# wgurecky/CORRLA_RS

Measured on AMD Instinct MI355X. Metric: RSVD GFLOP/s on 16k x 16k f32 rank-128, higher is better.
Workload: dtype f32

## Files before the change

### corrla_rs_amd/csrc/core_svd_plan.hpp

```cpp
#pragma once
#include <algorithm>
#include <cmath>
#include <cstddef>
#include <cstdint>
#include <cstring>
#include <limits>

#if defined(__HIPCC__)
#include <hip/hip_runtime.h>
#define CORRLA_HD __host__ __device__
#else
#define CORRLA_HD
#endif

namespace corrla {
namespace k {

constexpr size_t kLdsMaxBytes = (size_t)160 * 1024;

constexpr int kJmcMaxSweeps = 40;
constexpr int kJmcLanes = 16;
CORRLA_HD constexpr int jmc_rows(int nc, int lanes) { return nc * 2 * lanes; }
CORRLA_HD constexpr int jmc_pitch(int nc, int esz, int lanes) {
  return lanes == 8 ? (jmc_rows(nc, 8) + ((nc % 2 == 0) ? 16 : 0))
                    : (esz == 4 ? (jmc_rows(nc, 16) + ((nc % 2 == 0) ? 32 : 0)) : jmc_rows(nc, 16));
}
CORRLA_HD constexpr size_t jmc_lds_bytes(int nc, int b, int esz, int lanes) {
  return (size_t)2 * (2 * b) * jmc_pitch(nc, esz, lanes) * esz + (size_t)2 * b * esz + 64;
}

constexpr int kRingProcPad = 72;
constexpr int kReplayLanes = 16;
CORRLA_HD inline size_t jacobi_ring_w_lds_bytes(int l, int rs, size_t esz) {
  const int n2 = (l + 1) & ~1;
  const int nproc = n2 / 2;
  return (size_t)2 * nproc * rs * esz + (size_t)n2 * (esz + sizeof(int)) + (size_t)2 * nproc * esz + 64;
}
inline int jacobi_ring_e(int64_t l, int esz) { return l <= 64 ? 8 : (l <= 96 ? 12 : (l <= 128 ? 16 : (esz == 4 ? 20 : 18))); }

inline size_t jacobi_block_round_lds_bytes(int rows_pad, size_t esz) {
  return (size_t)(2 * 16 * (rows_pad + 1) + 7 * 16 * 17 + 32) * esz + 16 * sizeof(int) + 64;
}
inline size_t jacobi_finish_lds_bytes(int l, size_t esz) { return (size_t)(l + 2) * esz + (size_t)(l + 2) * sizeof(int) + 64; }

}

inline bool jmc_geometry(int64_t l, int esz, int jmc_max_b, int local, int np_force, int* nc_out, int* np_out, int* b_out) {
  if (l < 2 || l > 288) return false;
  const int nc = (int)((l + 2 * k::kJmcLanes - 1) / (2 * k::kJmcLanes));
  auto width = [&](int np_) {
    int bb = (int)((l + 2 * np_ - 1) / (2 * np_));
    return local ? (bb + 3) / 4 * 4 : bb + (bb & 1);
  };
  int np = np_force;
  if (np <= 0) {
    np = 2;
    while (np < 128 && (width(np) > jmc_max_b || k::jmc_lds_bytes(nc, width(np), esz, k::kJmcLanes) > k::kLdsMaxBytes)) ++np;
  }
  const int b = width(np);
  if (np < 1 || b < 2 || b > 32 || k::jmc_lds_bytes(nc, b, esz, k::kJmcLanes) > k::kLdsMaxBytes) return false;
  *nc_out = nc;
  *np_out = np;
  *b_out = b;
  return true;
}

enum class CoreSvd {
  kRing,
  kMultiWg,
  kBlock,
  kHost,
};
struct CoreSvdKnobs {
  const char* mode = nullptr;
  bool host_svd = false;
  int jmc_min_l = 96;
  int jmc_max_b = 24;
  int jmc_local = 1;
  int jmc_np = 0;
  int jmc_sweeps_f32 = 10, jmc_sweeps_f64 = 13;
  bool jmc_force_v = false;
  bool strict = false;
  int block_sweeps = 12, ring_sweeps = 40;
  int block_inner = 1;
};
struct CoreSvdState {
  int sweeps_hint = 0;
  int extra_sweeps = 0;
  bool force_v = false;
};

struct CoreSvdPlan {
  CoreSvd family = CoreSvd::kHost;
  int ring_e = 0;
  double tol = 0;
  double tol_early = 0;
  double floor2 = 0;
  struct MultiWg {
    int nc, np, b;
    int local;
    int rp;
    int nblocks, ncols_pad;
    unsigned step_threads;
    size_t step_lds;
    size_t ws_bytes;
    size_t fin_lds;
    unsigned other_grid;
    int force_v;
    int nsw;
    int group, max_sweeps;
  } mc = {};
  struct Block {
    int nb;
    int cols_pad, rows_pad;
    size_t ws_bytes;
    size_t round_lds;
    int max_sweeps, inner;
    size_t fin_lds;
  } blk = {};
  struct Ring {
    unsigned block;
    size_t lds;
    int max_sw;
    size_t rot_bytes, rank_bytes;
    unsigned replay_grid;
  } ring = {};
};

inline CoreSvdPlan core_svd_plan(int esz, int64_t l, int64_t k, const CoreSvdKnobs& kn, const CoreSvdState& st, bool optimistic) {
  auto is = [&](const char* m) { return kn.mode && std::strcmp(kn.mode, m) == 0; };
  CoreSvdPlan p;
  CoreSvdPlan::MultiWg& g = p.mc;
  const int e = k::jacobi_ring_e(l, esz);
  if ((!kn.mode || is("mc")) && !kn.host_svd && (is("mc") || l >= kn.jmc_min_l) &&
      jmc_geometry(l, esz, kn.jmc_max_b, kn.jmc_local, kn.jmc_np, &g.nc, &g.np, &g.b))
    p.family = CoreSvd::kMultiWg;
  else if (kn.host_svd || is("host") || l > 1024)
    return p;
  else if (!is("block") && l >= 2 && l <= 144 && k::jacobi_ring_w_lds_bytes((int)l, 8 * e, (size_t)esz) <= k::kLdsMaxBytes)
    p.family = CoreSvd::kRing;
  else
    p.family = CoreSvd::kBlock;

  const double eps = esz == 4 ? (double)std::numeric_limits<float>::epsilon() : std::numeric_limits<double>::epsilon();
  p.tol = std::sqrt((double)l) * eps;
  p.tol_early = kn.strict && p.family != CoreSvd::kBlock ? p.tol : std::sqrt(eps);
  p.floor2 = (double)l * eps * eps;
  switch (p.family) {
    case CoreSvd::kMultiWg: {
      g.local = kn.jmc_local;
      g.rp = k::jmc_pitch(g.nc, esz, k::kJmcLanes);
      g.nblocks = 2 * g.np;
      g.ncols_pad = g.nblocks * g.b;
      g.step_threads = (unsigned)((g.b * k::kJmcLanes + 63) / 64 * 64);
      g.step_lds = k::jmc_lds_bytes(g.nc, g.b, esz, k::kJmcLanes);
      g.ws_bytes = (size_t)g.rp * g.ncols_pad * esz;
      g.fin_lds = k::jacobi_finish_lds_bytes((int)l, (size_t)esz);
      g.other_grid = ((unsigned)(l * k) * 16 + 255) / 256;
      g.force_v = (!optimistic || st.force_v || kn.jmc_force_v) ? 1 : 0;
      const int nsw_default = std::max(1, esz == 4 ? kn.jmc_sweeps_f32 : kn.jmc_sweeps_f64);
      g.nsw = std::min(k::kJmcMaxSweeps, (st.sweeps_hint > 0 ? std::min(nsw_default, st.sweeps_hint + 2) : nsw_default) + st.extra_sweeps);
      g.group = 8;
      g.max_sweeps = k::kJmcMaxSweeps;
      break;
    }
    case CoreSvd::kBlock: {
      CoreSvdPlan::Block& b = p.blk;
      b.nb = (int)(2 * ((l + 15) / 16));
      b.cols_pad = b.nb * 8;
      b.rows_pad = (int)((l + 15) / 16 * 16);
      b.ws_bytes = (size_t)b.rows_pad * b.cols_pad * esz;
      b.round_lds = k::jacobi_block_round_lds_bytes(b.rows_pad, (size_t)esz);
      b.max_sweeps = kn.block_sweeps;
      b.inner = kn.block_inner;
      b.fin_lds = k::jacobi_finish_lds_bytes((int)l, (size_t)esz);
      break;
    }
    case CoreSvd::kRing: {
      CoreSvdPlan::Ring& r = p.ring;
      const int np = (int)((l + 1) / 2), n2 = 2 * np;
      p.ring_e = e;
      r.block = (unsigned)(np * 8);
      r.lds = k::jacobi_ring_w_lds_bytes((int)l, 8 * e, (size_t)esz);
      r.max_sw = kn.ring_sweeps;
      r.rot_bytes = (size_t)r.max_sw * n2 * k::kRingProcPad * (2 * (size_t)esz);
      r.rank_bytes = sizeof(int) * (size_t)n2;
      r.replay_grid = (unsigned)((l + 256 / k::kReplayLanes - 1) / (256 / k::kReplayLanes));
      break;
    }
    case CoreSvd::kHost: break;
  }
  return p;
}
inline CoreSvdPlan core_svd_plan(int esz, int64_t l, const CoreSvdKnobs& kn) { return core_svd_plan(esz, l, l, kn, CoreSvdState{}, true); }

}
```

### corrla_rs_amd/csrc/core_svd_stage.hpp

```cpp
#pragma once
#include "core_svd_plan.hpp"
#include "hip_backend.hpp"

namespace corrla {

template <class T>
struct CoreSvdCall {
  const Skinny<T>& c;
  int64_t l, k;
  Skinny<T>&m1, &m2;
  T* s_dev;
  void* conv_status;
};

namespace core_svd_stage {

template <class T>
using RingEs = std::integer_sequence<int, 8, 12, 16, sizeof(T) == 4 ? 20 : 18>;
constexpr int kMaxNc = 9;

template <class T>
inline void set_lds_limits() {
  for_each_of(RingEs<T>{}, [](auto e) { lds_limit((const void*)k::jacobi_ring_w_kernel<T, decltype(e)::value, 8>, k::kLdsMaxBytes); });
  lds_limit((const void*)k::jacobi_block_round_kernel<T>, k::kLdsMaxBytes);
  for_each_nt<kMaxNc>([](auto nc) { lds_limit((const void*)k::jmc_step_kernel<T, decltype(nc)::value, k::kJmcLanes>, k::kLdsMaxBytes); });
}

template <class T>
inline void multi_wg(HipDev& dev, const CoreSvdCall<T>& a, const CoreSvdPlan& plan) {
  const CoreSvdPlan::MultiWg& p = plan.mc;
  const int l = (int)a.l;
  T* wj = (T*)dev.alloc_bytes(p.ws_bytes);
  T* vj = (T*)dev.alloc_bytes(p.ws_bytes);
  k::JmcCtl* ctl = (k::JmcCtl*)dev.alloc_bytes(sizeof(k::JmcCtl));
  k::CholStatus* st = a.conv_status ? (k::CholStatus*)a.conv_status : (k::CholStatus*)dev.alloc_bytes(sizeof(k::CholStatus));
  hipLaunchKernelGGL((k::jmc_init_kernel<T>), dim3(1), dim3(1024), 0, dev.stream, (const T*)a.c.p, a.c.ld, l, wj, vj, p.rp,
                     p.ncols_pad, p.force_v, ctl);
  const T tol = (T)plan.tol, tol_early = (T)plan.tol_early, floor2 = (T)plan.floor2;
  auto enqueue_sweeps = [&](int s0, int s1) {
    for (int sw = s0; sw < s1; ++sw)
      for (int step = 0; step < p.nblocks - 1; ++step)
        with_nt<kMaxNc>(p.nc, [&](auto nc) {
          hipLaunchKernelGGL((k::jmc_step_kernel<T, decltype(nc)::value, k::kJmcLanes>), dim3((unsigned)p.np), dim3(p.step_threads),
                             p.step_lds, dev.stream, wj, vj, p.b, p.nblocks, step, sw, step == 0 ? 1 : 0, tol, tol_early, floor2,
                             ctl, p.local);
        });
    CORRLA_HIP(hipGetLastError());
  };
  auto finish = [&](int nsw) {
    hipLaunchKernelGGL((k::jmc_finish_kernel<T>), dim3(1), dim3(1024), p.fin_lds, dev.stream, (const T*)wj, (const T*)vj, p.rp, l,
                       nsw, (const k::JmcCtl*)ctl, a.m1.p, a.m1.ld, a.m2.p, a.m2.ld, a.s_dev, (int)a.k, st);
    hipLaunchKernelGGL((k::jmc_other_factor_kernel<T>), dim3(p.other_grid), dim3(256), 0, dev.stream, (const T*)a.c.p, a.c.ld, l,
                       (int)a.k, (const T*)a.m2.p, a.m2.ld, (const T*)a.s_dev, (const k::JmcCtl*)ctl, a.m1.p, a.m1.ld);
    CORRLA_HIP(hipGetLastError());
  };
  if (a.conv_status) {
    const int nsw = p.nsw;
    enqueue_sweeps(0, nsw);
    finish(nsw);
    if (env_int("CORRLA_DEBUG", 0)) {
      k::JmcCtl hd;
      CORRLA_HIP(hipMemcpyAsync(&hd, ctl, sizeof(hd), hipMemcpyDeviceToHost, dev.stream));
      dev.sync();
      int used = 0;
      while (used < nsw && hd.rot[used] && hd.big[used]) ++used;
      std::fprintf(stderr, "[corrla] jacobi_svd (multi-workgroup, %d sweeps enqueued, %s) l=%d np=%d b=%d nc=%d sweeps run=%d rounds(wg0)=%llu "
                           "cycles/round=%.0f ns/round=%.0f (%.0f MHz)\n", nsw, hd.with_v ? "V accumulated" : "W only", l, p.np, p.b, p.nc, std::min(used + 1, nsw),
                   hd.rounds, hd.rounds ? (double)hd.clk / hd.rounds : 0.0, hd.rounds ? 10.0 * hd.wall / hd.rounds : 0.0,
                   hd.wall ? 100.0 * hd.clk / hd.wall : 0.0);
      if (hd.steps)
        std::fprintf(stderr, "[corrla]   per step (wg0, us): load %.2f norms %.2f rounds %.2f store %.2f total %.2f over %llu steps\n",
                     0.01 * hd.t_load / hd.steps, 0.01 * hd.t_norm / hd.steps, 0.01 * hd.wall / hd.steps,
                     0.01 * hd.t_store / hd.steps, 0.01 * hd.t_total / hd.steps, hd.steps);
      if (hd.steps > 1)
        std::fprintf(stderr, "[corrla]   span first-start..last-end over all workgroups: %.2f us per step\n",
                     0.01 * hd.t_span / (hd.steps - 1));
    }
    return;
  }
  int done = 0;
  k::JmcCtl h;
  while (done < p.max_sweeps) {
    const int s1 = std::min(p.max_sweeps, done + p.group);
    enqueue_sweeps(done, s1);
    CORRLA_HIP(hipMemcpyAsync(&h, ctl, sizeof(h), hipMemcpyDeviceToHost, dev.stream));
    dev.sync();
    bool conv = false;
    for (int s_ = 0; s_ < s1; ++s_) conv = conv || !(h.rot[s_] && h.big[s_]);
    done = s1;
    if (conv || h.bad) break;
  }
  if (h.bad) throw Error(ST_ENUMERIC, "non-finite core matrix in small SVD");
  finish(done);
  if (env_int("CORRLA_DEBUG", 0)) {
    int used = 0;
    while (used < done && h.rot[used] && h.big[used]) ++used;
    std::fprintf(stderr, "[corrla] jacobi_svd (multi-workgroup) l=%d np=%d b=%d sweeps=%d\n", l, p.np, p.b, used + 1);
  }
}

template <class T>
inline void finite_check(HipDev& dev, const CoreSvdCall<T>& a) {
  int* bad = a.conv_status ? nullptr : dev.alloc_flags(1);
  hipLaunchKernelGGL((k::core_finite_check_kernel<T>), dim3(1), dim3(1024), 0, dev.stream, (const T*)a.c.p, a.c.ld, (int)a.l,
                     (k::CholStatus*)a.conv_status, bad);
  CORRLA_HIP(hipGetLastError());
  if (bad) {
    int h = 0;
    dev.read_flags(bad, 1, &h);
    if (h) throw Error(ST_ENUMERIC, "non-finite core matrix in small SVD");
  }
}

template <class T>
inline void block(HipDev& dev, const CoreSvdCall<T>& a, const CoreSvdPlan& plan) {
  const CoreSvdPlan::Block& p = plan.blk;
  const int64_t ld = p.rows_pad;
  T* wj = (T*)dev.alloc_bytes(p.ws_bytes);
  T* vj = (T*)dev.alloc_bytes(p.ws_bytes);
  k::JacobiCtl* ctl = (k::JacobiCtl*)dev.alloc_bytes(sizeof(k::JacobiCtl));
  hipLaunchKernelGGL((k::jacobi_init_kernel<T>), dim3(64), dim3(256), 0, dev.stream, (const T*)a.c.p, a.c.ld, (int)a.l, wj, ld, vj,
                     ld, p.cols_pad, p.rows_pad, ctl);
  for (int sw = 0; sw < p.max_sweeps; ++sw) {
    for (int round = 0; round < p.nb - 1; ++round)
      hipLaunchKernelGGL((k::jacobi_block_round_kernel<T>), dim3(p.nb / 2), dim3(256), p.round_lds, dev.stream, wj, ld, vj, ld,
                         p.rows_pad, p.nb, round, p.inner, ctl);
    hipLaunchKernelGGL(k::jacobi_sweep_end_kernel, dim3(1), dim3(1), 0, dev.stream, ctl, (float)plan.tol_early);
  }
  hipLaunchKernelGGL((k::jacobi_finish_kernel<T>), dim3(1), dim3(1024), p.fin_lds, dev.stream, (const T*)wj, ld, (const T*)vj,
                     ld, (int)a.l, a.m1.p, a.m1.ld, a.m2.p, a.m2.ld, a.s_dev, (int)a.k);
  CORRLA_HIP(hipGetLastError());
  if (env_int("CORRLA_DEBUG", 0)) {
    k::JacobiCtl h;
    CORRLA_HIP(hipMemcpyAsync(&h, ctl, sizeof(h), hipMemcpyDeviceToHost, dev.stream));
    dev.sync();
    std::fprintf(stderr, "[corrla] block jacobi l=%d nb=%d sweeps=%u done=%u\n", (int)a.l, p.nb, h.sweeps, h.done);
  }
}

template <class T>
inline void ring(HipDev& dev, const CoreSvdCall<T>& a, const CoreSvdPlan& plan) {
  static_assert(sizeof(k::RotEntry<T>) == 2 * sizeof(T), "CoreSvdPlan::Ring::rot_bytes");
  const CoreSvdPlan::Ring& p = plan.ring;
  int* info = (int*)dev.alloc_bytes(sizeof(int) * 4);
  k::RotEntry<T>* rot = (k::RotEntry<T>*)dev.alloc_bytes(p.rot_bytes);
  int* rank_g = (int*)dev.alloc_bytes(p.rank_bytes);
  const T tol = (T)plan.tol, tol_early = (T)plan.tol_early;
  with_one_of(RingEs<T>{}, plan.ring_e, [&](auto e) {
    hipLaunchKernelGGL((k::jacobi_ring_w_kernel<T, decltype(e)::value, 8>), dim3(1), dim3(p.block), p.lds, dev.stream, (const T*)a.c.p,
                       a.c.ld, (int)a.l, a.m2.p, a.m2.ld, a.s_dev, (int)a.k, tol, tol_early, p.max_sw, rot, rank_g, info);
  });
  CORRLA_HIP(hipGetLastError());
  hipLaunchKernelGGL((k::jacobi_replay_v_kernel<T>), dim3(p.replay_grid), dim3(256), 0, dev.stream, (const k::RotEntry<T>*)rot,
                     (const int*)info, (const int*)rank_g, (int)a.l, (int)a.k, a.m1.p, a.m1.ld);
  CORRLA_HIP(hipGetLastError());
  if (env_int("CORRLA_DEBUG", 0)) {
    int h[4] = {0, 0, 0, 0};
    CORRLA_HIP(hipMemcpyAsync(h, info, sizeof(int), hipMemcpyDeviceToHost, dev.stream));
    dev.sync();
    std::fprintf(stderr, "[corrla] jacobi_svd (ring) l=%d sweeps=%d\n", (int)a.l, h[0]);
  }
}

inline CoreSvdKnobs knobs_from_env() {
  CoreSvdKnobs kn;
  kn.mode = std::getenv("CORRLA_SVD");
  kn.host_svd = env_int("CORRLA_HOST_SVD", 0) != 0;
  kn.jmc_min_l = env_int("CORRLA_JMC_MIN_L", kn.jmc_min_l);
  kn.jmc_max_b = std::min(32, std::max(2, env_int("CORRLA_JMC_MAX_B", kn.jmc_max_b)));
  kn.jmc_local = env_int("CORRLA_JMC_LOCAL", kn.jmc_local);
  kn.jmc_np = env_int("CORRLA_JMC_NP", kn.jmc_np);
  kn.jmc_sweeps_f32 = env_int("CORRLA_JMC_SWEEPS", kn.jmc_sweeps_f32);
  kn.jmc_sweeps_f64 = env_int("CORRLA_JMC_SWEEPS", kn.jmc_sweeps_f64);
  kn.jmc_force_v = env_int("CORRLA_JMC_FORCE_V", 0) != 0;
  kn.strict = env_int("CORRLA_JACOBI_STRICT", 0) != 0;
  kn.block_sweeps = env_int("CORRLA_JACOBI_SWEEPS", kn.block_sweeps);
  kn.ring_sweeps = env_int("CORRLA_JACOBI_SWEEPS", kn.ring_sweeps);
  kn.block_inner = env_int("CORRLA_JACOBI_INNER", kn.block_inner);
  return kn;
}

}

template <class T>
void HipDev::small_svd(const Skinny<T>& c, int64_t l, int64_t k, Skinny<T>& m1, Skinny<T>& m2, T* s_dev, void* conv_status) {
  if (conv_status) memset_zero(conv_status, sizeof(k::CholStatus));
  const CoreSvdCall<T> a{c, l, k, m1, m2, s_dev, conv_status};
  const CoreSvdPlan plan = core_svd_plan((int)sizeof(T), l, k, core_svd_stage::knobs_from_env(), svd_state_, conv_status != nullptr);
  switch (plan.family) {
    case CoreSvd::kMultiWg:
      core_svd_stage::multi_wg(*this, a, plan);
      return;
    case CoreSvd::kHost:
      small_svd_host(*this, c, l, k, m1, m2, s_dev);
      return;
    case CoreSvd::kBlock:
      core_svd_stage::finite_check(*this, a);
      core_svd_stage::block(*this, a, plan);
      return;
    case CoreSvd::kRing:
      core_svd_stage::finite_check(*this, a);
      core_svd_stage::ring(*this, a, plan);
      return;
  }
}

}
```

### corrla_rs_amd/csrc/hip_backend.hpp

```cpp
#pragma once
#include <hip/hip_runtime.h>
#include <rccl/rccl.h>

#include <cmath>
#include <cstdio>
#include <cstdlib>
#include <cstring>
#include <limits>
#include <random>
#include <string>
#include <type_traits>
#include <utility>
#include <vector>

#include "core_svd_plan.hpp"
#include "driver.hpp"
#include "hip_kernels.hpp"
#include "tsqr_kernels.hpp"
#include "jacobi_mc_kernels.hpp"
#include "ata_kernels.hpp"
#include "tall_kernels.hpp"
#include "mixed_kernels.hpp"
#include "bf16in_kernels.hpp"
#include "grad_kernels.hpp"
// ... 589 lines not shown
    sync();
    std::memset(tmp, 0, n * sizeof(T));
    for (int64_t j = 0; j < cols; ++j)
      for (int64_t i = 0; i < rows; ++i) tmp[(size_t)j * dst.ld + i] = (T)host[(size_t)j * ld_host + i];
    CORRLA_HIP(hipMemcpyAsync(dst.p, tmp, n * sizeof(T), hipMemcpyHostToDevice, stream));
    if (!heap.empty()) sync();
  }
  template <class T>
  void upload_skinny_native(const T* host, int64_t ld_host, Skinny<T>& dst) {
    h2d_2d(dst.p, dst.ld, host, ld_host, dst.rows, dst.cols);
  }
  template <class T>
  void copy_in_skinny(const T* src_dev, int64_t ld_src, Skinny<T>& dst) {
    CORRLA_HIP(hipMemcpy2DAsync(dst.p, (size_t)dst.ld * sizeof(T), src_dev, (size_t)ld_src * sizeof(T),
                                (size_t)dst.rows * sizeof(T), (size_t)dst.cols, hipMemcpyDeviceToDevice, stream));
  }
  template <class T>
  void copy_skinny(const Skinny<T>& src, Skinny<T>& dst) {
    CORRLA_HIP(hipMemcpyAsync(dst.p, src.p, (size_t)src.ld * src.cols_alloc * sizeof(T), hipMemcpyDeviceToDevice, stream));
  }
  template <class T>
  void copy_cols(const Skinny<T>& src, Skinny<T>& dst, int64_t c0, int64_t n) {
    if (src.ld != dst.ld) throw Error(ST_EINVAL, "internal: copy_cols needs equal leading dimensions");
    if (n > 0)
      CORRLA_HIP(hipMemcpyAsync(dst.p + c0 * dst.ld, src.p, (size_t)n * src.ld * sizeof(T), hipMemcpyDeviceToDevice, stream));
  }
  template <class T>
  void sub_inplace(Skinny<T>& y, const Skinny<T>& p) {
    const int64_t n = y.ld * std::min(y.cols_alloc, p.cols_alloc);
    const int blocks = (int)std::min<int64_t>(4096, std::max<int64_t>(1, (n + 255) / 256));
    hipLaunchKernelGGL((k::sub_kernel<T>), dim3(blocks), dim3(256), 0, stream, y.p, (const T*)p.p, n);
    CORRLA_HIP(hipGetLastError());
  }
  template <class T>
  void zero_cols(Skinny<T>& s, int64_t c0, int64_t c1) {
    if (c1 > c0) memset_zero(s.p + c0 * s.ld, (size_t)(c1 - c0) * s.ld * sizeof(T));
  }
  template <class T>
  void store_values(const T* host_src, int64_t n, T* dst, bool dst_is_host) {
    if (dst_is_host) {
      std::memcpy(dst, host_src, sizeof(T) * n);
    } else {
      CORRLA_HIP(hipMemcpyAsync(dst, host_src, sizeof(T) * n, hipMemcpyHostToDevice, stream));
      sync();
    }
  }
  template <class T>
  void copy_values_out(const T* src_dev, int64_t n, T* dst, bool dst_is_host) {
    CORRLA_HIP(hipMemcpyAsync(dst, src_dev, sizeof(T) * n, dst_is_host ? hipMemcpyDeviceToHost : hipMemcpyDeviceToDevice,
                              stream));
    if (dst_is_host) sync();
  }
  template <class T>
  bool device_chol_fits(int64_t l) const {
    return l <= 4096 && k::chol_inv_fits((int)l, sizeof(T)) && !no_device_chol_;
  }
  template <class T>
  bool device_chol_blocked_fits(int64_t l) const {
    const int64_t n1 = round_up((l + 1) / 2, (int64_t)4);
    return l > 8 && l <= 4096 && k::chol_inv_fits((int)n1, sizeof(T)) && !no_device_chol_;
  }
  template <class T>
  void copy_block(const Skinny<T>& src, int64_t r0, int64_t c0, int64_t rows, int64_t cols, Skinny<T>& dst, int64_t dr0,
                  int64_t dc0) {
    if (rows <= 0 || cols <= 0) return;
    CORRLA_HIP(hipMemcpy2DAsync(dst.p + dc0 * dst.ld + dr0, (size_t)dst.ld * sizeof(T), src.p + c0 * src.ld + r0,
                                (size_t)src.ld * sizeof(T), (size_t)rows * sizeof(T), (size_t)cols, hipMemcpyDeviceToDevice,
                                stream));
  }
  template <class T>
  void chol_inv(const Skinny<T>& g, int64_t r, T piv_rel, Skinny<T>& m_out, void* st_dev, int slot) {
    hipLaunchKernelGGL((k::chol_inv_kernel<T>), dim3(1), dim3(k::chol_inv_threads((int)r)),
                       k::chol_inv_lds_bytes((int)r, sizeof(T)), stream, (const T*)g.p, g.ld, (int)r, piv_rel, m_out.p,
                       m_out.ld, (k::CholStatus*)st_dev + slot);
    CORRLA_HIP(hipGetLastError());
  }
  void set_run_if(const int* p) { run_if_ = p; }
  int robust_passes() const { return robust_passes_; }
  void set_robust_passes(int n) { robust_passes_ = n; }
  bool svd_more_sweeps() {
    if (svd_state_.extra_sweeps >= 24) return false;
    svd_state_.extra_sweeps += 8;
    svd_state_.sweeps_hint = 0;
    return true;
  }
  bool svd_force_v() {
    if (svd_state_.force_v) return false;
    svd_state_.force_v = true;
    return true;
  }
  void svd_sweeps_used(int n) { svd_state_.sweeps_hint = std::max(svd_state_.sweeps_hint - 1, n); }
  int* alloc_flags(int n) { return (int*)alloc_zeroed(sizeof(int) * (size_t)std::max(n, 1)); }
  void* alloc_zeroed_bytes(size_t bytes) { return alloc_zeroed(bytes); }
  void read_bytes(const void* dev_p, size_t bytes, void* host) {
    CORRLA_HIP(hipMemcpyAsync(host, dev_p, bytes, hipMemcpyDeviceToHost, stream));
    sync();
  }
  template <class T>
  void poison_entry(Skinny<T>& s, int64_t i, int64_t j, int kind) {
    hipLaunchKernelGGL((k::poison_entry_kernel<T>), dim3(1), dim3(1), 0, stream, s.p + j * s.ld + i, kind);
    CORRLA_HIP(hipGetLastError());
  }
  struct ArenaMark {
    std::vector<size_t> used, zused;
  };
  ArenaMark arena_mark() const {
    ArenaMark mk;
    for (const auto& c : chunks_) mk.used.push_back(c.used);
    for (const auto& c : zchunks_) mk.zused.push_back(c.used);
    return mk;
  }
  void arena_rewind(const ArenaMark& mk) {
    sp_scratch_ = nullptr;
    sp_scratch_bytes_ = 0;
    for (size_t i = 0; i < chunks_.size(); ++i) chunks_[i].used = i < mk.used.size() ? mk.used[i] : 0;
    for (size_t i = 0; i < zchunks_.size(); ++i) {
      Chunk& c = zchunks_[i];
      const size_t keep = i < mk.zused.size() ? mk.zused[i] : 0;
      if (c.used > keep) CORRLA_HIP(hipMemsetAsync((char*)c.p + keep, 0, c.used - keep, stream));
      c.zeroed = std::max(c.zeroed, c.used);
      c.used = keep;
    }
  }
  int sharded_handshake(int local_status) {
    if (comm_size <= 1 && !(comm && env_int("CORRLA_FORCE_ALLREDUCE", 0))) return local_status;
    if (!comm) throw Error(ST_ECOMM, "communicator not initialised");
    double h[8] = {(double)local_status, (double)robust_passes_, (double)svd_state_.extra_sweeps, (double)svd_state_.sweeps_hint,
                   svd_state_.force_v ? 1.0 : 0.0, 0.0, 0.0, 0.0};
    double* d = (double*)alloc_bytes(sizeof(h));
    CORRLA_HIP(hipMemcpyAsync(d, h, sizeof(h), hipMemcpyHostToDevice, stream));
    CORRLA_NCCL(ncclAllReduce(d, d, 8, ncclDouble, ncclMax, comm, stream));
    ++n_collectives;
    collective_bytes += sizeof(h);
    CORRLA_HIP(hipMemcpyAsync(h, d, sizeof(h), hipMemcpyDeviceToHost, stream));
    sync();
    robust_passes_ = (int)h[1];
    svd_state_.extra_sweeps = (int)h[2];
    svd_state_.sweeps_hint = (int)h[3];
    svd_state_.force_v = h[4] != 0.0;
    return (int)h[0];
  }
  void read_flags(const int* dev_p, int n, int* host) {
    CORRLA_HIP(hipMemcpyAsync(host, dev_p, sizeof(int) * (size_t)n, hipMemcpyDeviceToHost, stream));
    sync();
  }
  template <class T>
  bool device_qr_robust_fits(int64_t l) const {
    return robust_qr_ && (device_chol_fits<T>(l) || device_chol_blocked_fits<T>(l));
  }
  bool qr_inplace_fits(int64_t l) const { return col_blocking(l).nblk == 1; }
  template <class T>
  void* alloc_inspect() { return alloc_zeroed(sizeof(k::GramInspect<T>)); }
  template <class T>
  const void* inspect_shift_ptr(const void* insp) const { return &((const k::GramInspect<T>*)insp)->shift; }
  template <class T>
  void gram_inspect(Skinny<T>& g, int64_t l, float shift_rel, int shift_mode, void* insp) {
    hipLaunchKernelGGL((k::gram_inspect_kernel<T>), dim3(1), dim3(1024), 0, stream, g.p, g.ld, (int)l, shift_rel, shift_mode,
                       (k::GramInspect<T>*)insp, run_if_);
    CORRLA_HIP(hipGetLastError());
  }
  template <class T>
  void combine_need(int* need, const void* insp, const int* na, const int* nb) {
    hipLaunchKernelGGL((k::combine_need_kernel<T>), dim3(1), dim3(1), 0, stream, need, (const k::GramInspect<T>*)insp, na, nb,
                       run_if_);
    CORRLA_HIP(hipGetLastError());
  }
  template <class T>
  void chol_inv_robust(const Skinny<T>& g, int64_t r, T piv_rel, float shift_rel, int shift_mode, float null_excess,
                       Skinny<T>& m_out, void* st_dev, int slot, int* need_next, int* null_mask,
                       const void* abs_shift = nullptr, float need_ratio = 0.f) {
    k::CholRobust rb{shift_rel, shift_mode, null_excess, need_next, null_mask, run_if_, need_ratio, abs_shift};
    hipLaunchKernelGGL((k::chol_inv_kernel<T>), dim3(1), dim3(k::chol_inv_threads((int)r)),
                       k::chol_inv_lds_bytes((int)r, sizeof(T)), stream, (const T*)g.p, g.ld, (int)r, piv_rel, m_out.p,
                       m_out.ld, (k::CholStatus*)st_dev + slot, rb);
    CORRLA_HIP(hipGetLastError());
  }
  template <class T>
  void apply_inplace(Skinny<T>& y, int64_t l, const Skinny<T>& m) {
    Skinny<T> out = y.view_cols(l);
    Skinny<T> mv = m.view_cols(l);
    mv.rows = l;
    launch_gemm<T>(true, as_rowmajor_transposed(y, l), mv, out, (const T*)nullptr);
  }
  template <class T>
  void refill_null(Skinny<T>& y, int64_t l, const int* null_mask, uint64_t seed) {
    const int bx = (int)std::min<int64_t>(64, (y.rows + 255) / 256);
    hipLaunchKernelGGL((k::refill_null_kernel<T>), dim3((unsigned)std::max(bx, 1), (unsigned)l), dim3(256), 0, stream, y.p, y.ld,
                       y.rows, (int)l, null_mask, seed, run_if_);
    CORRLA_HIP(hipGetLastError());
  }

  void read_chol_status(const void* st_dev, int n, int* fail, float* min_ratio, float* dev_i) {
    static_assert(sizeof(k::CholStatus) == 32, "driver.hpp assumes 32-byte status records");
    static_assert(k::kNeedNonFinite == kFlagNonFinite && k::kNeedNullCols == kFlagNullCols, "need_next bits: kernels vs driver");
    std::vector<k::CholStatus> h((size_t)std::max(n, 1));
    CORRLA_HIP(hipMemcpyAsync(h.data(), st_dev, sizeof(k::CholStatus) * n, hipMemcpyDeviceToHost, stream));
    sync();
    for (int i = 0; i < n; ++i) {
      fail[i] = h[i].fail;
      min_ratio[i] = h[i].min_ratio;
      dev_i[i] = h[i].dev_i;
      if (env_int("CORRLA_DEBUG", 0) >= 2)
        std::fprintf(stderr, "[corrla] chol_inv[%d]: fail %d min_ratio %.3g dev_i %.3g clk %lld wall %lld (%.0f MHz)\n", i,
                     h[i].fail, h[i].min_ratio, h[i].dev_i, h[i].clk, h[i].wall,
                     h[i].wall > 0 ? 100.0 * (double)h[i].clk / (double)h[i].wall : 0.0);
    }
  }

  template <class T>
  void inv_sqrt_series(Skinny<T>& g, int64_t r, Skinny<T>& m_out) {
    Skinny<T> e2 = alloc_skinny<T>(r, r), e3 = alloc_skinny<T>(r, r);
    if (e2.ld != g.ld || m_out.ld != g.ld) throw Error(ST_EINVAL, "internal: series operands must share a leading dimension");
    dim3 grid((unsigned)((r + 63) / 64), (unsigned)r);
    hipLaunchKernelGGL((k::series_prep_kernel<T>), grid, dim3(64), 0, stream, g.p, g.ld, (int)r);
    Big<T> eb;
    eb.p = g.p;
    eb.rows = r;
    eb.cols = r;
    eb.ld = g.ld;
    eb.cols_readable = g.ld;
    Skinny<T> gv = g.view_cols(r);
    gv.rows = r;
// ... 340 lines not shown
    CORRLA_HIP(hipEventRecord(e, stream));
    marks_.push_back({e, slot});
  }
  void phase_forget() {
    for (auto& m_ : marks_) m_.slot = nullptr;
  }
  void phase_resolve(double* total) {
    for (size_t i = 1; i < marks_.size(); ++i) {
      float ms = 0.f;
      if (hipEventElapsedTime(&ms, marks_[i - 1].ev, marks_[i].ev) != hipSuccess) {
        (void)hipGetLastError();
        continue;
      }
      if (marks_[i].slot) *marks_[i].slot += (double)ms;
    }
    if (total && marks_.size() >= 2) {
      float ms = 0.f;
      if (hipEventElapsedTime(&ms, marks_.front().ev, marks_.back().ev) == hipSuccess)
        *total = (double)ms;
      else
        (void)hipGetLastError();
    }
    marks_.clear();
  }

  void event_mark(int i) {
    CORRLA_HIP(hipEventRecord(events_[i], stream));
    events_set_[i] = true;
  }
  double event_elapsed_ms(int i, int j) {
    if (!events_set_[i] || !events_set_[j]) return 0.0;
    float ms = 0.f;
    if (hipEventElapsedTime(&ms, events_[i], events_[j]) != hipSuccess) {
      (void)hipGetLastError();
      return 0.0;
    }
    return (double)ms;
  }

  template <class F>
  double time_on_stream(int reps, F&& f) {
    hipEvent_t e0, e1;
    CORRLA_HIP(hipEventCreate(&e0));
    CORRLA_HIP(hipEventCreate(&e1));
    f();
    CORRLA_HIP(hipEventRecord(e0, stream));
    for (int i = 0; i < reps; ++i) f();
    CORRLA_HIP(hipEventRecord(e1, stream));
    CORRLA_HIP(hipEventSynchronize(e1));
    float ms = 0.f;
    CORRLA_HIP(hipEventElapsedTime(&ms, e0, e1));
    (void)hipEventDestroy(e0);
    (void)hipEventDestroy(e1);
    return (double)ms / reps;
  }

 private:
  struct Chunk {
    void* p = nullptr;
    size_t size = 0, used = 0;
    size_t zeroed = 0;
  };
  std::vector<Chunk> chunks_;
  std::vector<Chunk> zchunks_;
  void* sp_scratch_ = nullptr;
  size_t sp_scratch_bytes_ = 0;
  void* zero_page_ = nullptr;
  void* pinned_ = nullptr;
  hipEvent_t events_[3] = {nullptr, nullptr, nullptr};
  bool events_set_[3] = {false, false, false};
  struct PhaseMark {
    hipEvent_t ev;
    double* slot;
  };
  std::vector<hipEvent_t> ev_pool_;
  size_t ev_used_ = 0;
  std::vector<PhaseMark> marks_;
  static constexpr size_t kPinnedBytes = (size_t)8 << 20;
  int gemm_debug_flags_ = 0;
  GemmKnobs gemm_knobs_;
  SyrkKnobs syrk_knobs_;
  uint64_t entropy_ = 0, calls_ = 0, calls_sharded_ = 0;
  bool no_device_chol_ = false;
  const int* run_if_ = nullptr;
  bool phase_events_ = true;
  bool robust_qr_ = true;
  int robust_passes_ = 2;
  CoreSvdState svd_state_;

  static void check_grid(const dim3& g) {
    if (g.y > 65535u || g.z > 65535u) throw Error(ST_EINVAL, "problem too large for the launch grid");
  }

  static void set_lds_limits() {
    constexpr size_t kMax = k::kLdsMaxBytes;
    set_lds_limits_typed<float>();
    set_lds_limits_typed<double>();
    core_svd_stage::set_lds_limits<float>();
    core_svd_stage::set_lds_limits<double>();
    set_ata_limits<2>();
    set_ata_limits<4>();
    set_ata_limits<8>();
    set_mixed_limits<2, false>();
    set_mixed_limits<2, true>();
    set_mixed_limits<3, false>();
    set_mixed_limits<3, true>();
    set_bf16a_limits();
    lds_limit((const void*)k::knn_kernel, kMax);
    lds_limit((const void*)k::knn_mfma_kernel<4, 4>, kMax);
    lds_limit((const void*)k::knn_mfma_kernel<4, 8>, kMax);
    lds_limit((const void*)k::knn_mfma_kernel<4, 16>, kMax);
    lds_limit((const void*)k::knn_mfma_kernel<2, 4>, kMax);
    lds_limit((const void*)k::knn_mfma_kernel<2, 8>, kMax);
    lds_limit((const void*)k::knn_mfma_kernel<2, 16>, kMax);
    lds_limit((const void*)k::knn2_kernel<1>, k::k2_lds_bytes(1));
    lds_limit((const void*)k::knn2_kernel<2>, k::k2_lds_bytes(2));
    lds_limit((const void*)k::grad_fit_kernel, kMax);
    lds_limit((const void*)k::grad_fit_lin_kernel<1>, kMax);
    lds_limit((const void*)k::grad_fit_lin_kernel<2>, kMax);
    lds_limit((const void*)k::grad_fit_lin_kernel<3>, kMax);
    lds_limit((const void*)k::grad_fit_lin_kernel<4>, kMax);
    lds_limit((const void*)k::grad_fit_lin_kernel<5>, kMax);
    lds_limit((const void*)k::knn_wide_kernel, k::ws_lds_bytes());
    lds_limit((const void*)k::grad_fit_wide_kernel, k::wf_lds_bytes());
  }
  template <class T>
  static void set_lds_limits_typed() {
    constexpr size_t kMax = k::kLdsMaxBytes;
    for_each_nt<kMaxColTiles>([](auto nt) { set_gemm_limits<T, decltype(nt)::value>(); });
    for_each_nt<sizeof(T) == 4 ? 6 : 4>([](auto nct) {
      lds_limit((const void*)k::tall_gram_kernel<T, decltype(nct)::value>, k::gram_lds_bytes(nct, (int)sizeof(T)));
    });
    lds_limit((const void*)k::syrk_kernel<T, true>, (size_t)k::syrk_lds_bytes((int)sizeof(T)));
    lds_limit((const void*)k::syrk_kernel<T, false>, (size_t)k::syrk_lds_bytes((int)sizeof(T)));
    lds_limit((const void*)k::hh_leaf_factor_kernel<T, false>, kMax);
    lds_limit((const void*)k::hh_tree_factor_kernel<T, false>, kMax);
    lds_limit((const void*)k::hh_tree_apply_kernel<T, false>, kMax);
    lds_limit((const void*)k::hh_leaf_apply_kernel<T, false>, kMax);
    lds_limit((const void*)k::hh_leaf_factor_kernel<T, true>, kMax);
    lds_limit((const void*)k::hh_tree_factor_kernel<T, true>, kMax);
    lds_limit((const void*)k::hh_tree_apply_kernel<T, true>, kMax);
    lds_limit((const void*)k::hh_leaf_apply_kernel<T, true>, kMax);
  }
  template <class T, int NT>
  static void set_gemm_limits() {
    lds_limit((const void*)k::gemm_nn_kernel<T, 1, NT>, k::gemm_lds_bytes(1, NT));
    lds_limit((const void*)k::gemm_tn_kernel<T, 1, NT>, k::gemm_lds_bytes(1, NT));
    lds_limit((const void*)k::gemm_nn_kernel<T, 2, NT>, k::gemm_lds_bytes(2, NT));
    lds_limit((const void*)k::gemm_tn_kernel<T, 2, NT>, k::gemm_lds_bytes(2, NT));
    if constexpr (NT <= 8) lds_limit((const void*)k::gemm_nn_kernel<T, 2, NT, true>, 3 * k::big_tile_bytes(2));
    if constexpr (std::is_same<T, double>::value) {
      lds_limit((const void*)k::gemm_nn_kernel<T, 1, NT, false, 8>, k::gemm_lds_bytes(2, NT));
      lds_limit((const void*)k::gemm_tn_kernel<T, 1, NT, 8>, k::gemm_lds_bytes(2, NT));
    }
  }
  template <int NK>
  static void set_ata_limits() {
    for_each_nt<5>([](auto nct) { lds_limit((const void*)k::ata_fused_kernel<NK, decltype(nct)::value>, k::ata_lds_bytes(NK, nct)); });
  }
  template <int NP, bool TN>
  static void set_mixed_limits() {
    for_each_nt<kMaxColTiles>([](auto nt) {
      lds_limit((const void*)k::gemm_bf16s_kernel<decltype(nt)::value, NP, TN>, k::mx_lds_bytes(nt, NP));
    });
  }
  static void set_bf16a_limits() {
// ... 108 lines not shown
```

### corrla_rs_amd/csrc/jacobi_mc_kernels.hpp

```cpp
#pragma once
#include "core_svd_plan.hpp"
#include "hip_kernels.hpp"

namespace corrla {
namespace k {

constexpr float kJmcFastCond = 16.f;
constexpr float kJmcVerifyCond = 64.f;
struct JmcCtl {
  unsigned rot[kJmcMaxSweeps + 1];
  unsigned big[kJmcMaxSweeps + 1];
  int sexp;
  int bad;
  int with_v;
  unsigned long long clk, wall;
  unsigned long long rounds;
  unsigned long long t_load, t_norm, t_store, t_total, steps;
  unsigned long long t_max_total;
  unsigned long long t_first, t_last;
  unsigned long long t_span;
};

template <class T>
struct JmcVec;
template <>
struct JmcVec<float> {
  typedef float v2 __attribute__((ext_vector_type(2)));
};
template <>
struct JmcVec<double> {
  typedef double v2 __attribute__((ext_vector_type(2)));
};

template <int LANES>
__device__ __forceinline__ float jmc_sum(float x) {
  return group_sum<LANES>(x);
}
template <int LANES>
__device__ __forceinline__ double jmc_sum(double x) {
  static_assert(LANES == 16, "f64 processors are 16 lanes wide");
  auto dpp = [](double v, auto ctrl) {
    int lo = __double2loint(v), hi = __double2hiint(v);
    lo = __builtin_amdgcn_update_dpp(0, lo, decltype(ctrl)::value, 0xf, 0xf, true);
    hi = __builtin_amdgcn_update_dpp(0, hi, decltype(ctrl)::value, 0xf, 0xf, true);
    return __hiloint2double(hi, lo);
  };
  x += dpp(x, std::integral_constant<int, 0xB1>{});
  x += dpp(x, std::integral_constant<int, 0x4E>{});
  x += dpp(x, std::integral_constant<int, 0x141>{});
  x += dpp(x, std::integral_constant<int, 0x140>{});
  return x;
}


template <class T>
__global__ __launch_bounds__(1024) void jmc_init_kernel(const T* __restrict__ c, int64_t ldc, int l, T* w, T* v, int rp,
                                                        int ncols_pad, int force_v, JmcCtl* ctl) {
  __shared__ float red[16];
  __shared__ int sbad;
  const int tid = threadIdx.x;
  if (tid == 0) sbad = 0;
  float mx = 0.f;
  int bad = 0;
  for (int idx0 = tid; idx0 < l * l; idx0 += 4 * 1024) {
    T xb[4];
#pragma unroll
    for (int u = 0; u < 4; ++u) {
      const int idx = min(idx0 + u * 1024, l * l - 1);
      const int j = idx / l, i = idx - j * l;
      xb[u] = c[(int64_t)j * ldc + i];
    }
#pragma unroll
    for (int u = 0; u < 4; ++u)
      if (idx0 + u * 1024 < l * l) {
        const float x = (float)fabs(xb[u]);
        if (!(x < 3.0e38f)) bad = 1;
        mx = fmaxf(mx, x);
      }
  }
  for (int off = 32; off > 0; off >>= 1) mx = fmaxf(mx, __shfl_xor(mx, off, 64));
  if ((tid & 63) == 0) red[tid >> 6] = mx;
  __syncthreads();
  if (bad) sbad = 1;
  mx = 0.f;
  for (int i = 0; i < 16; ++i) mx = fmaxf(mx, red[i]);
  __syncthreads();
  int sexp = 0;
  if (mx > 0.f && !sbad) {
    (void)frexpf(mx, &sexp);
    sexp = 1 - sexp;
  }
  const int total = rp * ncols_pad;
  for (int idx0 = tid; idx0 < total; idx0 += 4 * 1024) {
    T xb[4];
#pragma unroll
    for (int u = 0; u < 4; ++u) {
      const int idx = min(idx0 + u * 1024, total - 1);
      const int j = idx / rp, i = idx - j * rp;
      xb[u] = c[(int64_t)min(j, l - 1) * ldc + min(i, l - 1)];
    }
#pragma unroll
    for (int u = 0; u < 4; ++u) {
      const int idx = idx0 + u * 1024;
      if (idx < total) {
        const int j = idx / rp, i = idx - j * rp;
        const bool in = i < l && j < l;
        w[idx] = in ? (T)ldexp((double)xb[u], sexp) : (T)0;
        v[idx] = (in && i == j) ? (T)1 : (T)0;
      }
    }
  }
  for (int i = tid; i <= kJmcMaxSweeps; i += 1024) {
    ctl->rot[i] = 0;
    ctl->big[i] = 0;
  }
  float dmin = 3.0e38f, dmax = 0.f;
  for (int i = tid; i < l; i += 1024) {
    const float d = (float)fabs(c[(int64_t)i * ldc + i]);
    dmin = fminf(dmin, d);
    dmax = fmaxf(dmax, d);
  }
  for (int off = 32; off > 0; off >>= 1) {
    dmin = fminf(dmin, __shfl_xor(dmin, off, 64));
    dmax = fmaxf(dmax, __shfl_xor(dmax, off, 64));
  }
  __shared__ float rmin[16], rmax[16];
  if ((tid & 63) == 0) {
    rmin[tid >> 6] = dmin;
    rmax[tid >> 6] = dmax;
  }
  __syncthreads();
  if (tid == 0) {
    for (int i = 0; i < 16; ++i) {
      dmin = fminf(dmin, rmin[i]);
      dmax = fmaxf(dmax, rmax[i]);
    }
    ctl->with_v = (force_v || !(dmin * kJmcFastCond >= dmax) || !(dmax > 0.f)) ? 1 : 0;
    ctl->sexp = sexp;
    ctl->bad = sbad;
    ctl->clk = 0;
    ctl->wall = 0;
    ctl->rounds = 0;
    ctl->t_load = ctl->t_norm = ctl->t_store = ctl->t_total = ctl->steps = 0;
    ctl->t_max_total = ctl->t_span = 0;
    ctl->t_first = ~0ull;
    ctl->t_last = 0;
  }
}

__device__ __forceinline__ bool jmc_rotation_flat(float a, float b, float g, float tol, float tol_early, float floor2,
                                                  float& cs, float& sn, float& t, bool& big) {
  const float g2 = g * g, ab = a * b;
  const float zeta = (b - a) * 0.5f * __builtin_amdgcn_rcpf(g);
  const float den = fabsf(zeta) + __builtin_amdgcn_sqrtf(1.f + zeta * zeta);
  const float t_ = copysignf(__builtin_amdgcn_rcpf(den), zeta);
  const float c_ = __builtin_amdgcn_rsqf(1.f + t_ * t_);
  const float s_ = c_ * t_;
  const bool ok = (a > floor2) && (b > floor2) && (g2 > (tol * tol) * ab) && (fabsf(s_) <= 1.f) && (c_ <= 1.f);
  big = ok && (g2 > (tol_early * tol_early) * ab);
  cs = ok ? c_ : 1.f;
  sn = ok ? s_ : 0.f;
  t = ok ? t_ : 0.f;
  return ok;
}
__device__ __forceinline__ bool jmc_rotation_flat(double a, double b, double g, double tol, double tol_early, double floor2,
                                                  double& cs, double& sn, double& t, bool& big) {
  const double g2 = g * g, ab = a * b;
  const double zeta = (b - a) * 0.5 * jr_rcp(g);
  const double w = 1.0 + zeta * zeta;
  const double den = fabs(zeta) + w * jr_rsq(w);
  const double t_ = copysign(jr_rcp(den), zeta);
  const double c_ = jr_rsq(1.0 + t_ * t_);
  const double s_ = c_ * t_;
  const bool ok = (a > floor2) && (b > floor2) && (g2 > (tol * tol) * ab) && (fabs(s_) <= 1.0) && (c_ <= 1.0);
  big = ok && (g2 > (tol_early * tol_early) * ab);
  cs = ok ? c_ : 1.0;
  sn = ok ? s_ : 0.0;
  t = ok ? t_ : 0.0;
  return ok;
}

template <class T, int NC, int LANES>
__global__ __launch_bounds__(512) void jmc_step_kernel(T* w, T* v, int b, int nblocks, int step, int sweep, int within,
                                                        T tol, T tol_early, T floor2, JmcCtl* ctl, int local) {
  typedef typename JmcVec<T>::v2 v2;
  constexpr int PITCH = jmc_pitch(NC, (int)sizeof(T), LANES);
  const int sp = sweep > 0 ? sweep - 1 : 0;
  const unsigned rot_prev = ctl->rot[sp], big_prev = ctl->big[sp];
  const int bad_in = ctl->bad, with_v_in = ctl->with_v;
  if (sweep > 0 && !(rot_prev && big_prev)) return;
  if (bad_in) return;
  if (threadIdx.x == 0 && blockIdx.x == 0 && ctl->t_last != 0) {
    ctl->t_span += ctl->t_last - ctl->t_first;
    ctl->t_first = ~0ull;
    ctl->t_last = 0;
  }
  extern __shared__ __attribute__((aligned(16))) char smem[];
  T* wl = (T*)smem;
// ... 473 lines not shown
```

Measured before the change: 93760.

## Parallelize Jacobi init across blocks, fold status clear, adapt sweep margin

The single-block Jacobi init kernel now runs on up to 16 blocks for the workspace fill. Only block 0 does the control setup, and it also zeroes the convergence status, which removes a separate memset launch on the multi-WG path. A separate change tightens the sweep margin from 2 to 1 once the measured sweep count has repeated, so fewer Jacobi sweeps get enqueued. Fewer sweeps risk leaving a rank-128 core SVD unconverged and triggering the retry path; every block also recomputes the max-reduction redundantly.

```diff
diff --git a/corrla_rs_amd/csrc/core_svd_plan.hpp b/corrla_rs_amd/csrc/core_svd_plan.hpp
--- a/corrla_rs_amd/csrc/core_svd_plan.hpp
+++ b/corrla_rs_amd/csrc/core_svd_plan.hpp
@@ -86,6 +86,7 @@
 };
 struct CoreSvdState {
   int sweeps_hint = 0;
+  int sweeps_margin = 2;
   int extra_sweeps = 0;
   bool force_v = false;
 };
@@ -159,7 +160,7 @@
       g.other_grid = ((unsigned)(l * k) * 16 + 255) / 256;
       g.force_v = (!optimistic || st.force_v || kn.jmc_force_v) ? 1 : 0;
       const int nsw_default = std::max(1, esz == 4 ? kn.jmc_sweeps_f32 : kn.jmc_sweeps_f64);
-      g.nsw = std::min(k::kJmcMaxSweeps, (st.sweeps_hint > 0 ? std::min(nsw_default, st.sweeps_hint + 2) : nsw_default) + st.extra_sweeps);
+      g.nsw = std::min(k::kJmcMaxSweeps, (st.sweeps_hint > 0 ? std::min(nsw_default, st.sweeps_hint + st.sweeps_margin) : nsw_default) + st.extra_sweeps);
       g.group = 8;
       g.max_sweeps = k::kJmcMaxSweeps;
       break;
diff --git a/corrla_rs_amd/csrc/core_svd_stage.hpp b/corrla_rs_amd/csrc/core_svd_stage.hpp
--- a/corrla_rs_amd/csrc/core_svd_stage.hpp
+++ b/corrla_rs_amd/csrc/core_svd_stage.hpp
@@ -34,8 +34,8 @@
   T* vj = (T*)dev.alloc_bytes(p.ws_bytes);
   k::JmcCtl* ctl = (k::JmcCtl*)dev.alloc_bytes(sizeof(k::JmcCtl));
   k::CholStatus* st = a.conv_status ? (k::CholStatus*)a.conv_status : (k::CholStatus*)dev.alloc_bytes(sizeof(k::CholStatus));
-  hipLaunchKernelGGL((k::jmc_init_kernel<T>), dim3(1), dim3(1024), 0, dev.stream, (const T*)a.c.p, a.c.ld, l, wj, vj, p.rp,
-                     p.ncols_pad, p.force_v, ctl);
+  hipLaunchKernelGGL((k::jmc_init_kernel<T>), dim3(k::jmc_init_grid(p.rp * p.ncols_pad)), dim3(1024), 0, dev.stream,
+                     (const T*)a.c.p, a.c.ld, l, wj, vj, p.rp, p.ncols_pad, p.force_v, ctl, a.conv_status ? st : (k::CholStatus*)nullptr);
   const T tol = (T)plan.tol, tol_early = (T)plan.tol_early, floor2 = (T)plan.floor2;
   auto enqueue_sweeps = [&](int s0, int s1) {
     for (int sw = s0; sw < s1; ++sw)
@@ -184,9 +184,9 @@
 
 template <class T>
 void HipDev::small_svd(const Skinny<T>& c, int64_t l, int64_t k, Skinny<T>& m1, Skinny<T>& m2, T* s_dev, void* conv_status) {
-  if (conv_status) memset_zero(conv_status, sizeof(k::CholStatus));
   const CoreSvdCall<T> a{c, l, k, m1, m2, s_dev, conv_status};
   const CoreSvdPlan plan = core_svd_plan((int)sizeof(T), l, k, core_svd_stage::knobs_from_env(), svd_state_, conv_status != nullptr);
+  if (conv_status && plan.family != CoreSvd::kMultiWg) memset_zero(conv_status, sizeof(k::CholStatus));
   switch (plan.family) {
     case CoreSvd::kMultiWg:
       core_svd_stage::multi_wg(*this, a, plan);
diff --git a/corrla_rs_amd/csrc/hip_backend.hpp b/corrla_rs_amd/csrc/hip_backend.hpp
--- a/corrla_rs_amd/csrc/hip_backend.hpp
+++ b/corrla_rs_amd/csrc/hip_backend.hpp
@@ -695,6 +695,8 @@
     if (svd_state_.extra_sweeps >= 24) return false;
     svd_state_.extra_sweeps += 8;
     svd_state_.sweeps_hint = 0;
+    svd_state_.sweeps_margin = 2;
+    sweeps_last_ = sweeps_same_ = 0;
     return true;
   }
   bool svd_force_v() {
@@ -702,7 +704,12 @@
     svd_state_.force_v = true;
     return true;
   }
-  void svd_sweeps_used(int n) { svd_state_.sweeps_hint = std::max(svd_state_.sweeps_hint - 1, n); }
+  void svd_sweeps_used(int n) {
+    svd_state_.sweeps_hint = std::max(svd_state_.sweeps_hint - 1, n);
+    sweeps_same_ = n == sweeps_last_ ? sweeps_same_ + 1 : 1;
+    sweeps_last_ = n;
+    svd_state_.sweeps_margin = sweeps_same_ >= 2 ? 1 : 2;
+  }
   int* alloc_flags(int n) { return (int*)alloc_zeroed(sizeof(int) * (size_t)std::max(n, 1)); }
   void* alloc_zeroed_bytes(size_t bytes) { return alloc_zeroed(bytes); }
   void read_bytes(const void* dev_p, size_t bytes, void* host) {
@@ -739,7 +746,7 @@
     if (comm_size <= 1 && !(comm && env_int("CORRLA_FORCE_ALLREDUCE", 0))) return local_status;
     if (!comm) throw Error(ST_ECOMM, "communicator not initialised");
     double h[8] = {(double)local_status, (double)robust_passes_, (double)svd_state_.extra_sweeps, (double)svd_state_.sweeps_hint,
-                   svd_state_.force_v ? 1.0 : 0.0, 0.0, 0.0, 0.0};
+                   svd_state_.force_v ? 1.0 : 0.0, (double)svd_state_.sweeps_margin, 0.0, 0.0};
     double* d = (double*)alloc_bytes(sizeof(h));
     CORRLA_HIP(hipMemcpyAsync(d, h, sizeof(h), hipMemcpyHostToDevice, stream));
     CORRLA_NCCL(ncclAllReduce(d, d, 8, ncclDouble, ncclMax, comm, stream));
@@ -751,6 +758,7 @@
     svd_state_.extra_sweeps = (int)h[2];
     svd_state_.sweeps_hint = (int)h[3];
     svd_state_.force_v = h[4] != 0.0;
+    svd_state_.sweeps_margin = (int)h[5];
     return (int)h[0];
   }
   void read_flags(const int* dev_p, int n, int* host) {
@@ -1257,6 +1265,7 @@
   SyrkKnobs syrk_knobs_;
   uint64_t entropy_ = 0, calls_ = 0, calls_sharded_ = 0;
   bool no_device_chol_ = false;
+  int sweeps_last_ = 0, sweeps_same_ = 0;
   const int* run_if_ = nullptr;
   bool phase_events_ = true;
   bool robust_qr_ = true;
diff --git a/corrla_rs_amd/csrc/jacobi_mc_kernels.hpp b/corrla_rs_amd/csrc/jacobi_mc_kernels.hpp
--- a/corrla_rs_amd/csrc/jacobi_mc_kernels.hpp
+++ b/corrla_rs_amd/csrc/jacobi_mc_kernels.hpp
@@ -53,9 +53,13 @@
 }
 
 
+__host__ __device__ inline unsigned jmc_init_grid(int total) {
+  const int nb = (total + 4095) / 4096;
+  return (unsigned)(nb < 1 ? 1 : (nb > 16 ? 16 : nb));
+}
 template <class T>
 __global__ __launch_bounds__(1024) void jmc_init_kernel(const T* __restrict__ c, int64_t ldc, int l, T* w, T* v, int rp,
-                                                        int ncols_pad, int force_v, JmcCtl* ctl) {
+                                                        int ncols_pad, int force_v, JmcCtl* ctl, CholStatus* clear_st) {
   __shared__ float red[16];
   __shared__ int sbad;
   const int tid = threadIdx.x;
@@ -91,7 +95,7 @@
     sexp = 1 - sexp;
   }
   const int total = rp * ncols_pad;
-  for (int idx0 = tid; idx0 < total; idx0 += 4 * 1024) {
+  for (int idx0 = (int)blockIdx.x * 4 * 1024 + tid; idx0 < total; idx0 += (int)gridDim.x * 4 * 1024) {
     T xb[4];
 #pragma unroll
     for (int u = 0; u < 4; ++u) {
@@ -110,10 +114,12 @@
       }
     }
   }
+  if (blockIdx.x != 0) return;
   for (int i = tid; i <= kJmcMaxSweeps; i += 1024) {
     ctl->rot[i] = 0;
     ctl->big[i] = 0;
   }
+  if (clear_st && tid < (int)(sizeof(CholStatus) / sizeof(int))) ((int*)clear_st)[tid] = 0;
   float dmin = 3.0e38f, dmax = 0.f;
   for (int i = tid; i < l; i += 1024) {
     const float d = (float)fabs(c[(int64_t)i * ldc + i]);
```

Measured after the change: 94210, median of 2. Within noise of the previous version (+0.5%).
